# Celebrandil/CudaSift

Hardware: AMD Instinct MI355X
Metric: 1920x1080 SIFT frames/sec (higher is better)
Workload: dtype f32

## Files before the change

### cudasift_amd/csrc/chain.hpp

```cpp
#pragma once
#include "common.hpp"

#define CHAIN_MAX_LEVELS 3
struct ChainLevel { int w, h, p; long long off; };
struct ChainGeom {
  int K, T, tiles_x, tiles_y;
  long long frame_stride;
  ChainLevel lv[CHAIN_MAX_LEVELS + 1];
};

static inline int chain_lds_floats(int K, int T)
{
  const int n1 = ((T + 3) << (K - 1)) - 3, n0 = ((T + 3) << K) - 3;
  return n0 * n0 + n0 * n1 + n1 * n1;
}
#define CHAIN_LDS_FLOATS_MAX (85 * 85 + 85 * 41 + 41 * 41)
#define CHAIN_LDS_FLOATS_EMBED (53 * 53 + 53 * 25 + 25 * 25)

#ifdef __HIPCC__
__device__ __forceinline__ void scaledown_chain_block(float *__restrict__ scratch, const ChainGeom &G, const Taps5 &t,
                                                      int tile, int frame_index, float *lds)
{
  const int lane = threadIdx.x & 63, wave = threadIdx.x >> 6, nwaves = blockDim.x >> 6;
  const int tx = tile % G.tiles_x, ty = tile / G.tiles_x;
  float *frame = scratch + (long long)frame_index * G.frame_stride;
  const float k0 = t.k[0], k1 = t.k[1], k2 = t.k[2];
  auto ax = [&](int k) -> int { return (tx * G.T - 2) * (1 << (G.K - k)) + 2; };
  auto ay = [&](int k) -> int { return (ty * G.T - 2) * (1 << (G.K - k)) + 2; };
  auto n = [&](int k) -> int { return ((G.T + 3) << (G.K - k)) - 3; };
  float *const s_a = lds, *const s_h = lds + n(0) * n(0), *const s_b = s_h + n(0) * n(1);
  {
    const ChainLevel &S = G.lv[0];
    const float *src = frame + S.off;
    const int n0 = n(0), ax0 = ax(0), ay0 = ay(0);
// ... 56 lines not shown
```

### cudasift_amd/csrc/common.hpp

```cpp
#pragma once
#include <hip/hip_runtime.h>
#include <stdint.h>
#include <stddef.h>
#include "misift.h"

#define NUM_SCALES 5
#define NUM_BLURS  8
#define NUM_DOG    7
#define CNT_STRIDE 64
#define CNT_MAXPTS 17
#define CNT_CAND   20
#define CNT_CANDOVF 28
#define CNT_PTOVF  29
#define CNT_CHAINTMO 30
#define CNT_DET    32
#define CNT_DUP    40
#define CNT_SPARE_BLOCKS 9
#define CNT_BIG    48
#define CNT_TICKET 49
#define CNT_ORIDONE 50
#define CNT_FUSETMO 31

struct alignas(16) SiftPointD {
  float xpos, ypos, scale, sharpness, edgeness, orientation, score, ambiguity;
  int   match;
  float match_xpos, match_ypos, match_error, subsampling;
  float empty[3];
  float data[128];
};
static_assert(sizeof(SiftPointD) == MISIFT_POINT_BYTES, "record size");

struct BatchLayout {
  SiftPointD *recs;
  const int *counts, *offsets;
  int stride;
// ... 281 lines not shown
  float *d_own_scratch;
  size_t own_scratch_floats;
  int lds_pad_lpd, lds_pad_scan, lds_pad_orient, lds_pad_descr;
  float patch_reach;
  int fold_descr_tail;
  int descr_big_fallbacks;
  PendingBig pending_big;
  unsigned *d_refcap;
  size_t refcap_bytes;
  unsigned *d_capcnt;
  size_t capcnt_bytes;
  int refcap_limit;
  void *d_match_tmp;
  size_t match_tmp_bytes;
  int num_cus;
  int split_tail, in_capture;
  hipStream_t stream2;
  hipEvent_t ev_fork, ev_join;
  int *pack_counts, *pack_offsets;
  SiftPointD *pack_dst;
  int orient_blocks_per_cu;
  int point_blocks_per_cu;
  int strip_waves_per_cu, scan_waves_per_cu;
  int chain_max_frames;
  int chain_embed;
  unsigned chain_wait_ticks;
  int chain_fallbacks;
  int fuse_orient;
  unsigned fuse_wait_ticks;
  int fuse_fallbacks;
  int bin_min_frames;
  int small_frames;
  int lowpass_tile;
  int strip_rows_small;
  int scan_rows_small_coarse;
  int scan_rows_small;
  int cur_binned;
  int balance_frames;
  int cur_balanced;
  int4 *d_block_map;
// ... 131 lines not shown
```

### cudasift_amd/csrc/kernels_dog.hip

```cpp
#include <stdlib.h>
#include <string.h>
#include <math.h>
#include "common.hpp"
#include "chain.hpp"

#define WAVES_PER_BLOCK 4
#define OUT_LANES 62

struct ItemCoord { int frame, strip, seg; bool valid; };

__device__ __forceinline__ ItemCoord decode_item(const StripGeom &g)
{
  const unsigned lb = (g.noremap & 1) ? blockIdx.x : xcd_remap(blockIdx.x, gridDim.x);
  const int wave = __builtin_amdgcn_readfirstlane((int)(threadIdx.x >> 6));
  const long long item = (long long)lb * WAVES_PER_BLOCK + wave;
  const long long nitems = (long long)g.nframes * g.nstrips * g.nsegs;
  ItemCoord c;
  c.valid = item < nitems;
  if (g.noremap & 2) {
    c.strip = (int)(item % g.nstrips);
    const long long r = item / g.nstrips;
    c.seg = (int)(r % g.nsegs);
    c.frame = (int)(r / g.nsegs);
  } else {
// ... 840 lines not shown
  unsigned cap_clear_words;
  ScanOct o[MISIFT_MAX_OCTAVES];
};

#ifndef SCAN_OCC
#define SCAN_OCC (SCAN_RING ? 4 : 3)
#endif
#ifndef SCAN_STAMPS
#define SCAN_STAMPS 0
#endif
#if SCAN_STAMPS
#define STAMP_MAX(slot) do { if ((threadIdx.x & 63) == 0) atomicMax(&counters[(size_t)G.nframes * CNT_STRIDE + (slot)], (unsigned)wall_clock64()); } while (0)
#else
#define STAMP_MAX(slot) do { } while (0)
#endif
template <int FAST, bool CHAIN>
__global__ __launch_bounds__(256, SCAN_OCC) void dog_scan_all_kernel(const float *__restrict__ scratch, ScanAllGeom G,
                                                              AllTaps taps, float thresh,
                                                              unsigned *__restrict__ counters,
                                                              unsigned *__restrict__ cand, ChainGeom C, Taps5 k5,
                                                              int nchain)
{
  __shared__ v2f s_taps[WAVES_PER_BLOCK][NUM_SCAN_PAIRS * 5];
#if SCAN_RING
  __shared__ float4 s_win[WAVES_PER_BLOCK][RING_FLOAT4S];
  static_assert(sizeof(float4) * WAVES_PER_BLOCK * RING_FLOAT4S >= sizeof(float) * CHAIN_LDS_FLOATS_EMBED,
                "the chain borrows the scan's row ring");
#else
  __shared__ float s_chain_lds[CHAIN ? CHAIN_LDS_FLOATS_EMBED : 4];
#endif
// ... 6 lines not shown
  const int wave = __builtin_amdgcn_readfirstlane((int)(threadIdx.x >> 6));
  const int lane = threadIdx.x & 63;
  bool chain_failed = false;
  float4 *xch = nullptr;
#if SCAN_XCH && SCAN_XCH_DPP < 3
  if (lane < 4) s_xch[wave][(lane >> 1) * XCH_PLANE + (lane & 1) * (XCH_PLANE - 1)] = make_float4(0.f, 0.f, 0.f, 0.f);
  xch = &s_xch[wave][lane];
#endif
  if (CHAIN) {
#if SCAN_STAMPS
    if (blockIdx.x == 0 && threadIdx.x == 0) counters[(size_t)G.nframes * CNT_STRIDE + 8] = (unsigned)wall_clock64();
    if (threadIdx.x == 0) STAMP_MAX(14);
    if (threadIdx.x == 0 && lb + 1 == gridDim.x) STAMP_MAX(16);
    if (threadIdx.x == 0 && lb == (unsigned)nchain) STAMP_MAX(17);
#endif
    if (lb < (unsigned)nchain) {
      const int tiles = C.tiles_x * C.tiles_y;
#if SCAN_RING
      float *chain_lds = reinterpret_cast<float *>(&s_win[0][0]);
#else
      float *chain_lds = s_chain_lds;
#endif
      scaledown_chain_block(const_cast<float *>(scratch), C, k5, (int)(lb % tiles), (int)(lb / tiles), chain_lds);
      asm volatile("s_waitcnt vmcnt(0)" ::: "memory");
      __builtin_amdgcn_fence(__ATOMIC_RELEASE, "workgroup");
      __syncthreads();
      STAMP_MAX(9);
      if (threadIdx.x == 0) {
        unsigned *spare = counters + (size_t)G.nframes * CNT_STRIDE;
        const unsigned sub = lb & 15u, members = ((unsigned)nchain - sub + 15u) / 16u;
        if (atomicAdd(&spare[64 + 32 * sub], 1u) == members - 1u) {
          const unsigned nsub = (unsigned)nchain < 16u ? (unsigned)nchain : 16u;
          if (atomicAdd(&spare[32], 1u) == nsub - 1u && G.wait_ticks != 0u) {
            __hip_atomic_fetch_or(&spare[0], 0x80000000u, __ATOMIC_RELAXED, __HIP_MEMORY_SCOPE_AGENT);
            STAMP_MAX(18);
          }
        }
      }
      STAMP_MAX(19);
      return;
    }
    lb -= (unsigned)nchain;
    if (G.wait_lev < G.nlev && (long long)lb * WAVES_PER_BLOCK + (WAVES_PER_BLOCK - 1) >= G.o[G.wait_lev].item_begin) {
      STAMP_MAX(15);
      __shared__ unsigned s_chain_ok;
      if (threadIdx.x == 0) {
        const unsigned long long t0 = wall_clock64();
        unsigned ok = 1u;
        while ((__hip_atomic_fetch_add(&counters[(size_t)G.nframes * CNT_STRIDE], 1u, __ATOMIC_RELAXED, __HIP_MEMORY_SCOPE_AGENT) &
                0x80000000u) == 0u) {
          if (wall_clock64() - t0 > (unsigned long long)G.wait_ticks) { ok = 0u; break; }
          __builtin_amdgcn_s_sleep(8);
        }
        if (!ok) atomicAdd(&counters[CNT_CHAINTMO], 1u);
        s_chain_ok = ok;
      }
      __syncthreads();
      STAMP_MAX(13);
// ... 586 lines not shown
    const CapLayout L = cap_layout(P);
    const int rc = ensure_capcnt(ctx, P, L);
    if (rc) return rc;
    G.cap_clear = ctx->d_capcnt;
    G.cap_clear_words = L.words * (unsigned)P.nframes;
  }
  const AllTaps at = pack_taps(taps, P.noct);
  ChainGeom C;
  Taps5 t5;
  memset(&C, 0, sizeof(C));
  memset(&t5, 0, sizeof(t5));
  int nchain = 0;
  if (chain) {
    C = *chain;
    for (int j = 0; j < 5; j++) t5.k[j] = k5[j];
    nchain = C.tiles_x * C.tiles_y * P.nframes;
    G.wait_lev = 0;
    G.wait_ticks = ctx->chain_wait_ticks;
    for (int k = 0; k < G.nlev; k++)
      if (G.o[k].img_off == C.lv[0].off) G.wait_lev = k + 1;
  }
  const dim3 grid((unsigned)((items + WAVES_PER_BLOCK - 1) / WAVES_PER_BLOCK) + (unsigned)nchain);
  LaunchScope ls(ctx, "dog_scan");
#define SCAN_LAUNCH(F, CH) hipLaunchKernelGGL((dog_scan_all_kernel<F, CH>), grid, dim3(256), (size_t)ctx->lds_pad_scan, ctx->stream, scratch, G, at, \
                                              thresh, ctx->d_counters, ctx->d_cand, C, t5, nchain)
  if (chain) {
    if (fast && !ragged) SCAN_LAUNCH(1, true);
    else if (fast) SCAN_LAUNCH(2, true);
    else SCAN_LAUNCH(0, true);
  } else {
    if (fast && !ragged) SCAN_LAUNCH(1, false);
    else if (fast) SCAN_LAUNCH(2, false);
    else SCAN_LAUNCH(0, false);
  }
#undef SCAN_LAUNCH
// ... 41 lines not shown
```

### cudasift_amd/csrc/kernels_pyramid.hip

```cpp
#include <string.h>
#include "common.hpp"
#include "chain.hpp"

#define WAVES_PER_BLOCK 4
#define OUT_LANES 62

struct ItemCoord { int frame, strip, seg; bool valid; };

__device__ __forceinline__ ItemCoord decode_item(const StripGeom &g)
{
  const unsigned lb = (g.noremap & 1) ? blockIdx.x : xcd_remap(blockIdx.x, gridDim.x);
  const int wave = __builtin_amdgcn_readfirstlane((int)(threadIdx.x >> 6));
  const long long item = (long long)lb * WAVES_PER_BLOCK + wave;
  const long long nitems = (long long)g.nframes * g.nstrips * g.nsegs;
  ItemCoord c;
  c.valid = item < nitems;
  if (g.noremap & 2) {
    c.strip = (int)(item % g.nstrips);
    const long long r = item / g.nstrips;
    c.seg = (int)(r % g.nsegs);
    c.frame = (int)(r / g.nsegs);
  } else {
    c.seg = (int)(item % g.nsegs);
    const long long r = item / g.nsegs;
// ... 360 lines not shown
    const float *c = s_DH + (2 * Y) * (LPT_TW / 2) + X;
    float v = __builtin_fmaf(d2, c[2 * (LPT_TW / 2)], d0 * (c[0] + c[4 * (LPT_TW / 2)]));
    v = __builtin_fmaf(d1, c[LPT_TW / 2] + c[3 * (LPT_TW / 2)], v);
    LPT_STORE1(out2 + (size_t)Yg * dpitch2 + Xg, v);
  }
}

template <int FAST>
__global__ __launch_bounds__(256) void scaledown_kernel(const float *__restrict__ src, StripGeom g,
                                                        float *__restrict__ dst, int dpitch,
                                                        long long dst_frame_stride, Taps5 t, int src_aligned,
                                                        int dst_aligned)
{
  const ItemCoord it = decode_item(g);
  if (!it.valid) return;
  const int lane = threadIdx.x & 63;
  const int q = it.strip * OUT_LANES + lane - 1;
  const int w2 = g.width / 2, h2 = g.height / 2;
  const float *img = src + (long long)it.frame * g.frame_stride;
  float *out = dst + (long long)it.frame * dst_frame_stride;
  const int y0 = it.seg * g.seg_rows;
  const int y1 = min(y0 + g.seg_rows, h2);
  const float k0 = t.k[0], k1 = t.k[1], k2 = t.k[2];
  const bool sal = src_aligned != 0, dal = dst_aligned != 0;

  const QuadCol qa = make_quadcol(2 * q, g.width), qb = make_quadcol(2 * q + 1, g.width);
  struct Raw2 { float4 A, B; };
  auto ldraw = [&](int y) -> Raw2 {
    const float *row = img + (size_t)clampi(y, 0, g.height - 1) * g.pitch;
    Raw2 r;
    r.A = load_quad_t<FAST>(row, 2 * q, g.width, sal, qa);
    r.B = load_quad_t<FAST>(row, 2 * q + 1, g.width, sal, qb);
    return r;
  };
  auto hfilt = [&](const Raw2 &rw) -> float4 {
    const float4 A = rw.A, B = rw.B;
    const float lz = lane_from_left(B.z), lw = lane_from_left(B.w);
    const float rx = lane_from_right(A.x);
    float4 h;
    float s;
    s = __builtin_fmaf(k0, lz + A.z, k1 * (lw + A.y));  h.x = __builtin_fmaf(k2, A.x, s);
    s = __builtin_fmaf(k0, A.x + B.x, k1 * (A.y + A.w)); h.y = __builtin_fmaf(k2, A.z, s);
    s = __builtin_fmaf(k0, A.z + B.z, k1 * (A.w + B.y)); h.z = __builtin_fmaf(k2, B.x, s);
    s = __builtin_fmaf(k0, B.x + rx, k1 * (B.y + B.w)); h.w = __builtin_fmaf(k2, B.z, s);
    return h;
  };
  auto vcomb = [&](float a0, float a1, float a2, float a3, float a4) -> float {
    float s = __builtin_fmaf(k2, a2, k0 * (a0 + a4));
    s = __builtin_fmaf(k1, a1 + a3, s);
    return s;
  };

  auto hrow = [&](int y) -> float4 { return hfilt(ldraw(y)); };
  const bool writer = lane >= 1 && lane <= OUT_LANES && 4 * q < w2;
  const bool fast_store = FAST && (w2 & 3) == 0 && dal;
  float4 t0 = hrow(2 * y0 - 2), t1 = hrow(2 * y0 - 1), t2 = hrow(2 * y0), t3, t4;
  Raw2 ra = ldraw(2 * y0 + 1), rb = ldraw(2 * y0 + 2), rc = ldraw(2 * y0 + 3), rd = ldraw(2 * y0 + 4);
  for (int y = y0; y < y1; y++) {
    const Raw2 na = ldraw(2 * y + 5), nb = ldraw(2 * y + 6);
    t3 = hfilt(ra);
    t4 = hfilt(rb);
    ra = rc; rb = rd; rc = na; rd = nb;
    float4 o;
    o.x = vcomb(t0.x, t1.x, t2.x, t3.x, t4.x);
    o.y = vcomb(t0.y, t1.y, t2.y, t3.y, t4.y);
    o.z = vcomb(t0.z, t1.z, t2.z, t3.z, t4.z);
    o.w = vcomb(t0.w, t1.w, t2.w, t3.w, t4.w);
    if (writer) {
      if (fast_store) *reinterpret_cast<float4 *>(out + (size_t)y * dpitch + 4 * q) = o;
      else store_quad(out + (size_t)y * dpitch, q, w2, dal, o);
    }
    t0 = t2; t1 = t3; t2 = t4;
  }
}

__global__ __launch_bounds__(1024) void scaledown_chain_kernel(float *__restrict__ scratch, ChainGeom G, Taps5 t)
{
  __shared__ float s_lds[CHAIN_LDS_FLOATS_MAX];
  scaledown_chain_block(scratch, G, t, (int)blockIdx.x, (int)blockIdx.y, s_lds);
}

template <typename SRC>
__global__ __launch_bounds__(256) void scaleup_kernel(const SRC *__restrict__ src0, int w, int h, int spitch,
                                                      long long src_frame_stride, float *__restrict__ dst0, int dpitch,
                                                      long long dst_frame_stride)
{
  const int x = blockIdx.x * 64 + (threadIdx.x & 63);
  const int y = blockIdx.y * 4 + (threadIdx.x >> 6);
// ... 167 lines not shown
```

### cudasift_amd/csrc/misift_host.hip

```cpp
#include <stdarg.h>
#include <stdio.h>
#include <stdlib.h>
#include <string.h>
#include <math.h>
#include <initializer_list>
#include <map>
#include <mutex>
#include <string>
#include <utility>
#include <vector>
#include "common.hpp"
#include "chain.hpp"
#include "pair_plan.hpp"

static thread_local char g_err[512] = "";

void misift_set_error(const char *fmt, ...)
{
  va_list ap;
  va_start(ap, fmt);
  vsnprintf(g_err, sizeof(g_err), fmt, ap);
  va_end(ap);
}

// ... 260 lines not shown
  {"lds_pad_descr", "MISIFT_LDS_PAD_DESCR"}, {"lowpass_tile", "MISIFT_LOWPASS_TILE"}, {"strip_rows_small", "MISIFT_STRIP_ROWS_SMALL"},
  {"scan_rows_small_coarse", "MISIFT_SCAN_ROWS_SMALL_COARSE"}, {"scan_rows_small", "MISIFT_SCAN_ROWS_SMALL"},
  {"host_spin", "MISIFT_HOST_SPIN"}, {"refcap_limit", "MISIFT_TEST_REFCAP_LIMIT"}, {"fuse_orient", "MISIFT_FUSE_ORIENT"},
  {"fuse_wait_us", "MISIFT_FUSE_WAIT_US"},
};
static bool tunables_from_env()
{
  const char *e = getenv("MISIFT_TUNABLES");
  return e && atoi(e) != 0;
}
static int apply_knob(misift_ctx *ctx, const char *name, double v)
{
  const int i = (int)v;
  const auto is = [&](const char *n) { return strcmp(name, n) == 0; };
  if (is("graph")) extra(ctx)->graph_mode = i != 0;
  else if (is("split_tail")) ctx->split_tail = i;
  else if (is("bin")) ctx->bin_detections = i != 0;
  else if (is("descr_occ")) ctx->descr_occ = i;
  else if (is("tile")) ctx->tile_descr = ctx->tile_orient = i != 0;
  else if (is("tile_descr")) ctx->tile_descr = i != 0;
  else if (is("tile_orient")) ctx->tile_orient = i != 0;
  else if (is("orient_blocks")) ctx->orient_blocks_per_cu = i > 0 ? i : 6;
  else if (is("point_blocks")) ctx->point_blocks_per_cu = i > 0 ? i : 8;
  else if (is("strip_waves")) ctx->strip_waves_per_cu = i > 0 ? i : 16;
  else if (is("scan_waves")) ctx->scan_waves_per_cu = i > 0 ? i : 16;
  else if (is("chain_frames")) ctx->chain_max_frames = i;
  else if (is("chain_embed")) ctx->chain_embed = i != 0;
  else if (is("chain_wait_us")) ctx->chain_wait_ticks = (unsigned)(v * 100.0);
  else if (is("bin_min_frames")) ctx->bin_min_frames = i;
  else if (is("small_frames")) ctx->small_frames = i;
  else if (is("balance")) ctx->balance_frames = i != 0;
// ... 22 lines not shown
    for (const KnobName &k : KNOBS) all += std::string(all.empty() ? "" : ",") + k.name + "=" + k.env;
  return all.c_str();
}

extern "C" void misift_ctx_destroy(misift_ctx *ctx);
static int ctx_init(misift_ctx *ctx, CtxFull *f, int device, void *stream)
{
  ctx->device = device;
  ctx->stream = (hipStream_t)stream;
  default_options_full(&ctx->opt);
  hipDeviceProp_t prop;
  HIP_TRY(hipGetDeviceProperties(&prop, device));
  ctx->num_cus = prop.multiProcessorCount > 0 ? prop.multiProcessorCount : 256;
  ctx->strip_waves_per_cu = 32;
  ctx->scan_waves_per_cu = 32;
  ctx->split_tail = 8;
  {
    int lo = 0, hi = 0;
    HIP_TRY(hipDeviceGetStreamPriorityRange(&lo, &hi));
    HIP_TRY(hipStreamCreateWithPriority(&ctx->stream2, hipStreamNonBlocking, hi));
    HIP_TRY(hipEventCreateWithFlags(&ctx->ev_fork, hipEventDisableTiming));
    HIP_TRY(hipEventCreateWithFlags(&ctx->ev_join, hipEventDisableTiming));
  }
  ctx->bin_detections = 1;
  ctx->descr_occ = 4;
  ctx->tile_descr = 1;
  ctx->tile_orient = 0;
  ctx->orient_blocks_per_cu = 6;
  ctx->point_blocks_per_cu = 8;
  ctx->chain_max_frames = 4;
  ctx->chain_embed = 1;
  ctx->chain_wait_ticks = 10000000u;
  ctx->bin_min_frames = 4;
  ctx->small_frames = 4;
  ctx->balance_frames = 1;
  ctx->fold_descr_tail = 1;
  ctx->fuse_orient = 0;
  ctx->fuse_wait_ticks = 10000000u;
  ctx->patch_reach = 17.9f;
  ctx->refcap_limit = 32;
  ctx->lowpass_tile = 1;
  ctx->strip_rows_small = 6;
  ctx->scan_rows_small_coarse = 2;
  ctx->scan_rows_small = 4;
  ctx->host_spin = 0;
  if (tunables_from_env()) {
// ... 193 lines not shown
  if (x->d_mb_plan) misift_dev_free(x->d_mb_plan);
  if (ctx->d_counters) misift_dev_free(ctx->d_counters);
  if (ctx->h_counters) hipHostFree(ctx->h_counters);
  if (ctx->d_flags) misift_dev_free(ctx->d_flags);
  if (ctx->h_flags) hipHostFree(ctx->h_flags);
  if (ctx->d_cand) misift_dev_free(ctx->d_cand);
  if (ctx->d_det) misift_dev_free(ctx->d_det);
  if (ctx->d_det_sorted) misift_dev_free(ctx->d_det_sorted);
  if (ctx->d_block_map) misift_dev_free(ctx->d_block_map);
  if (ctx->d_own_scratch) misift_dev_free(ctx->d_own_scratch);
  if (ctx->d_match_tmp) misift_dev_free(ctx->d_match_tmp);
  if (ctx->d_refcap) misift_dev_free(ctx->d_refcap);
  if (ctx->d_capcnt) misift_dev_free(ctx->d_capcnt);
  if (ctx->ev0) hipEventDestroy(ctx->ev0);
  if (ctx->ev1) hipEventDestroy(ctx->ev1);
  if (ctx->stream2) { hipStreamSynchronize(ctx->stream2); hipStreamDestroy(ctx->stream2); }
  if (ctx->ev_fork) hipEventDestroy(ctx->ev_fork);
  if (ctx->ev_join) hipEventDestroy(ctx->ev_join);
  if (x->own_stream) hipStreamDestroy(x->own_stream);
  delete reinterpret_cast<CtxFull *>(ctx);
}

extern "C" int misift_ctx_set_graph_replay(misift_ctx *ctx, int on)
{
  ARG_CHECK(ctx != nullptr);
  extra(ctx)->graph_mode = on ? 1 : 0;
  return MISIFT_OK;
}

extern "C" int misift_ctx_set_stream(misift_ctx *ctx, void *stream)
{
  ARG_CHECK(ctx != nullptr);
  ctx->stream = (hipStream_t)stream;
// ... 555 lines not shown
      L.img_off = (long long)(lv[o].img - d_scratch);
      L.subsampling = (float)(1 << (num_octaves - o));
      L.lowest_scale = lowest_scale / L.subsampling;
      size_t c = (size_t)L.w * L.h / 4;
      if (c < 16384) c = 16384;
      L.cand_cap = (unsigned)c;
      L.cand_off = off;
      off += L.cand_cap;
      tapsv[o] = octave_taps(table, o);
    }
    rc = misift_ensure_frames(ctx, nframes, off);
    if (rc) return rc;
    rc = ensure_det(ctx, nframes, max_pts);
    if (rc) return rc;
  }
  bool scanned = false;
  if (ctx->opt.fused && ctx->split_tail && nframes >= ctx->split_tail && !ctx->in_capture && first_down_done &&
      num_octaves >= 3 && ctx->stream2) {
    HIP_TRY(hipEventRecord(ctx->ev_fork, ctx->stream));
    HIP_TRY(hipStreamWaitEvent(ctx->stream2, ctx->ev_fork, 0));
    rc = launch_dog_scan_all(ctx, d_scratch, P, tapsv.data(), thresh, 0, 2);
    if (rc) return rc;
    hipStream_t saved = ctx->stream;
    ctx->stream = ctx->stream2;
    for (int o = num_octaves - 1; o >= 2 && !rc; o--) {
      const Level &src = lv[o], &dst = lv[o - 1];
      StripGeom g = make_geom(ctx, src.w, src.h, src.p, nframes, SS, dst.w, dst.h, 62);
      rc = launch_scaledown(ctx, src.img, g, dst.img, dst.p, SS, k5);
    }
    if (!rc) rc = launch_dog_scan_all(ctx, d_scratch, P, tapsv.data(), thresh, 2, num_octaves);
    ctx->stream = saved;
    if (rc) return rc;
    HIP_TRY(hipEventRecord(ctx->ev_join, ctx->stream2));
    HIP_TRY(hipStreamWaitEvent(ctx->stream, ctx->ev_join, 0));
    scanned = true;
  }
  const bool chained = !scanned && !tiny && nframes <= ctx->chain_max_frames;
  ChainGeom embed;
  bool embedded = false;
  if (chained && ctx->opt.fused && ctx->chain_embed && ctx->want_export && first_down_done && num_octaves >= 3 &&
      num_octaves - 2 <= 3) {
    const int o = num_octaves - 1, nlev = o - 1;
    int dims[4][3];
    long long offs[4];
    for (int k = 0; k <= nlev; k++) {
      dims[k][0] = lv[o - k].w; dims[k][1] = lv[o - k].h; dims[k][2] = lv[o - k].p;
      offs[k] = (long long)(lv[o - k].img - d_scratch);
    }
    rc = make_chain_geom(&embed, SS, dims, offs, nlev, 4);
    if (rc) return rc;
    embedded = true;
  }
  for (int o = num_octaves; o >= 2 && !scanned && !embedded;) {
    if (o == num_octaves && first_down_done) { o--; continue; }
    if (chained) {
      const int nlev = (o - 1) < 3 ? (o - 1) : 3;
      int dims[4][3];
      long long offs[4];
      for (int k = 0; k <= nlev; k++) {
        dims[k][0] = lv[o - k].w; dims[k][1] = lv[o - k].h; dims[k][2] = lv[o - k].p;
        offs[k] = (long long)(lv[o - k].img - d_scratch);
      }
      rc = launch_scaledown_chain(ctx, d_scratch, SS, nframes, dims, offs, nlev, k5);
      if (rc) return rc;
      o -= nlev;
      continue;
    }
    const Level &src = lv[o], &dst = lv[o - 1];
    if (dst.w < 1 || dst.h < 1) break;
    StripGeom g = make_geom(ctx, src.w, src.h, src.p, nframes, SS, dst.w, dst.h, 62);
    rc = launch_scaledown(ctx, src.img, g, dst.img, dst.p, SS, k5);
    if (rc) return rc;
    o--;
  }
  if (ctx->opt.fused) {
    if (!scanned) {
      rc = launch_dog_scan_all(ctx, d_scratch, P, tapsv.data(), thresh, 0, num_octaves, embedded ? &embed : nullptr, k5);
      if (rc) return rc;
    }
    rc = launch_refine_all(ctx, d_scratch, P, tapsv.data(), thresh, 10.0f, 1.0f / NUM_SCALES, max_pts);
    if (rc) return rc;
    const bool binned = (ctx->bin_detections && nframes >= ctx->bin_min_frames) || ctx->opt.deterministic;
    ctx->cur_binned = binned ? 1 : 0;
    ctx->cur_balanced = 0;
    if (binned) {
      rc = launch_bin_detections(ctx, P, max_pts);
      if (rc) return rc;
    }
    if (ctx->fuse_orient && !binned && !ctx->pack_dst && nframes <= ctx->small_frames && ctx->tile_descr && !ctx->tile_orient &&
        !ctx->in_capture)
      return launch_orient_descr_fused(ctx, d_scratch, P, pts, max_pts);
    rc = launch_orient_all(ctx, d_scratch, P, pts, max_pts);
    if (rc) return rc;
    if (ctx->opt.deterministic) {
// ... 78 lines not shown
    if (ctx->pending_big.valid) {
      bool any = false;
      for (int f = 0; f < nframes; f++) any = any || ctx->h_counters[(size_t)f * CNT_STRIDE + CNT_BIG] != 0;
      if (!any) ctx->pending_big.valid = 0;
      else {
        rc = launch_descr_big_pending(ctx);
        if (!rc) rc = wait_host_flag(ctx, ctx->h_counters + (size_t)nframes * CNT_STRIDE, ctx->export_seq);
        if (rc) return rc;
      }
    }
  } else {
    HIP_TRY(hipMemcpyAsync(ctx->h_counters, ctx->d_counters, sizeof(unsigned) * CNT_STRIDE * (size_t)nframes,
                           hipMemcpyDeviceToHost, ctx->stream));
    HIP_TRY(hipStreamSynchronize(ctx->stream));
  }
  if (ctx->h_counters[CNT_CHAINTMO]) return MISIFT_RETRY_CHAIN;
  if (ctx->h_counters[CNT_FUSETMO]) return MISIFT_RETRY_FUSE;
  const int slot = 2 * num_octaves + (ctx->opt.fix_numpts ? 1 : 0);
  for (int f = 0; f < nframes; f++) {
    const unsigned c = ctx->h_counters[(size_t)f * CNT_STRIDE + slot];
    num_pts_out[f] = (int)(c < (unsigned)max_pts ? c : (unsigned)max_pts);
    if (ctx->h_counters[(size_t)f * CNT_STRIDE + CNT_CANDOVF]) *cand_overflow = true;
  }
  return MISIFT_OK;
}

static int enqueue_via_graph(misift_ctx *ctx, const CallKey &key, const void *d_imgs, long long frame_stride,
                             float *d_scratch, SiftPointD *pts)
{
  CtxExtra *x = extra(ctx);
  if (!x->graph_mode || ctx->profile || !d_scratch || key.scale_up || !key.fused) return 0;
// ... 851 lines not shown
```

### cudasift_amd/csrc/pipeline.hip

```cpp
#include <string.h>
#include <vector>
#include "common.hpp"

__global__ __launch_bounds__(1024) void export_counts_kernel(const unsigned *__restrict__ counters, int nframes, int slot,
                                                              int max_pts, int *__restrict__ counts,
                                                              int *__restrict__ offsets, int staged_noct)
{
  __shared__ int wave_tot[16];
  __shared__ int carry_s;
  const int tid = threadIdx.x, lane = tid & 63, wave = tid >> 6;
  if (tid == 0) carry_s = 0;
  __syncthreads();
  for (int f0 = 0; f0 < nframes; f0 += 1024) {
    const int f = f0 + tid;
    int c = 0;
    if (f < nframes) {
      const unsigned *cnt = counters + (size_t)f * CNT_STRIDE;
      unsigned n = cnt[slot];
      if (staged_noct > 0) {
        n = 0;
        for (int k = 1; k <= staged_noct; k++) {
          n += cnt[CNT_DET + k];
          if (k < staged_noct || (slot & 1)) n += cnt[CNT_DUP + k];
        }
      }
      c = (int)(n < (unsigned)max_pts ? n : (unsigned)max_pts);
      counts[f] = cnt[CNT_CANDOVF] ? -1 : c;
      if (cnt[CNT_CANDOVF]) c = 0;
    }
    if (!offsets) continue;
    int incl = c;
    for (int d = 1; d < 64; d <<= 1) {
      const int o = __shfl_up(incl, d, 64);
      if (lane >= d) incl += o;
    }
    if (lane == 63) wave_tot[wave] = incl;
    __syncthreads();
    int base = carry_s;
    for (int w = 0; w < wave; w++) base += wave_tot[w];
    if (f < nframes) offsets[f] = base + incl - c;
    __syncthreads();
    if (tid == 1023) carry_s = base + incl;
    __syncthreads();
// ... 159 lines not shown
    misift_set_error("misift_pipe_submit: invalid argument");
    return MISIFT_EINVAL;
  }
  if (p->submitted - p->collected >= p->depth) {
    misift_set_error("misift_pipe_submit: all %d slots are in flight — collect a batch first", p->depth);
    return MISIFT_EINVAL;
  }
  misift_ctx *ctx = p->ctx;
  HIP_TRY(hipSetDevice(ctx->device));
  PipeSlot &s = p->slots[p->submitted % p->depth];
  const size_t elem = p->src_u8 ? 1 : sizeof(float);
  HIP_TRY(hipMemcpyAsync(s.d_frames, host_frames, elem * p->frame_elems * nframes, hipMemcpyHostToDevice, p->s_up));
  HIP_TRY(hipEventRecord(s.ev_uploaded, p->s_up));
  HIP_TRY(hipStreamWaitEvent(p->s_compute, s.ev_uploaded, 0));
  hipStream_t saved = ctx->stream;
  const int saved_split = ctx->split_tail;
  ctx->stream = p->s_compute;
  ctx->split_tail = 0;
  const int fused_saved = ctx->opt.fused;
  if (misift_tiny_call(p->width, p->height, p->num_octaves)) ctx->opt.fused = 0;
  int rc = misift_extract_enqueue(ctx, s.d_frames, p->src_u8, nframes, (long long)p->frame_elems, p->width, p->height,
                                  p->width, p->num_octaves, p->init_blur, p->thresh, p->lowest_scale, 0, p->d_scratch,
                                  p->d_pts, p->max_pts);
  if (!rc) rc = launch_export_counts(ctx, nframes, p->num_octaves, p->max_pts, s.d_counts, s.d_counts + p->batch);
  if (!rc) rc = launch_pack_records(ctx, p->d_pts, p->max_pts, nframes, s.d_counts + p->batch, s.d_packed);
  ctx->stream = saved;
  ctx->split_tail = saved_split;
  ctx->opt.fused = fused_saved;
  if (rc) return rc;
  HIP_TRY(hipEventRecord(s.ev_done, p->s_compute));
  HIP_TRY(hipStreamWaitEvent(p->s_down, s.ev_done, 0));
  HIP_TRY(hipMemcpyAsync(s.h_counts, s.d_counts, sizeof(int) * (2 * (size_t)p->batch + 1), hipMemcpyDeviceToHost,
                         p->s_down));
  HIP_TRY(hipEventRecord(s.ev_counts, p->s_down));
  s.nframes = nframes;
  p->submitted++;
  return MISIFT_OK;
}

extern "C" int misift_pipe_collect(misift_pipe *p, int *nframes_out, int *counts_out, void *host_records,
                                   size_t capacity_records, size_t *nrecords_out)
{
// ... 72 lines not shown
```

Before: 58000.

## Embed staged scaledown chain into DoG scan launch, replacing second-stream split tail

Removes the two-stream split-tail path that forked the lower-octave scaledowns and scans onto a high-priority stream. For large batches it now embeds the lower-octave scaledowns as extra workgroups in the first DoG scan launch. These workgroups run in stages, and each stage waits on per-frame completion flags and tickets before reading the level above it. The scaledown body is factored into a shared device function with a write-through store variant. This removes separate kernel launches and event syncs, at the cost of spin-waiting workgroups, a timeout fallback reported per frame, and a dependence on workgroup scheduling order.

```diff
diff --git a/cudasift_amd/csrc/chain.hpp b/cudasift_amd/csrc/chain.hpp
--- a/cudasift_amd/csrc/chain.hpp
+++ b/cudasift_amd/csrc/chain.hpp
@@ -3,11 +3,17 @@
 
 #define CHAIN_MAX_LEVELS 3
 struct ChainLevel { int w, h, p; long long off; };
+struct ChainStage { int nstrips, nsegs, seg_rows; unsigned wg_begin; };
 struct ChainGeom {
   int K, T, tiles_x, tiles_y;
+  int staged;
+  int nwg;
   long long frame_stride;
   ChainLevel lv[CHAIN_MAX_LEVELS + 1];
+  ChainStage st[CHAIN_MAX_LEVELS];
 };
+#define CHAIN_FLAG_DONE 0x80000000u
+#define CHAIN_FLAG_FAILED 0x40000000u
 
 static inline int chain_lds_floats(int K, int T)
 {
@@ -18,6 +24,87 @@
 #define CHAIN_LDS_FLOATS_EMBED (53 * 53 + 53 * 25 + 25 * 25)
 
 #ifdef __HIPCC__
+#define SD_OUT_LANES 62
+typedef float sd_v4f __attribute__((ext_vector_type(4)));
+template <bool WT>
+__device__ __forceinline__ void sd_store1(float *p, float v)
+{
+  if (WT) __hip_atomic_store(p, v, __ATOMIC_RELAXED, __HIP_MEMORY_SCOPE_AGENT);
+  else *p = v;
+}
+template <int FAST, bool WT>
+__device__ __forceinline__ void scaledown_item(const float *__restrict__ img, int width, int height, int pitch,
+                                               float *__restrict__ out, int dpitch, int strip, int y0, int y1,
+                                               const Taps5 &t, bool sal, bool dal)
+{
+  const int lane = threadIdx.x & 63;
+  const int q = strip * SD_OUT_LANES + lane - 1;
+  const int w2 = width / 2;
+  const float k0 = t.k[0], k1 = t.k[1], k2 = t.k[2];
+
+  const QuadCol qa = make_quadcol(2 * q, width), qb = make_quadcol(2 * q + 1, width);
+  struct Raw2 { float4 A, B; };
+  auto ldraw = [&](int y) -> Raw2 {
+    const float *row = img + (size_t)clampi(y, 0, height - 1) * pitch;
+    Raw2 r;
+    r.A = load_quad_t<FAST>(row, 2 * q, width, sal, qa);
+    r.B = load_quad_t<FAST>(row, 2 * q + 1, width, sal, qb);
+    return r;
+  };
+  auto hfilt = [&](const Raw2 &rw) -> float4 {
+    const float4 A = rw.A, B = rw.B;
+    const float lz = lane_from_left(B.z), lw = lane_from_left(B.w);
+    const float rx = lane_from_right(A.x);
+    float4 h;
+    float s;
+    s = __builtin_fmaf(k0, lz + A.z, k1 * (lw + A.y));  h.x = __builtin_fmaf(k2, A.x, s);
+    s = __builtin_fmaf(k0, A.x + B.x, k1 * (A.y + A.w)); h.y = __builtin_fmaf(k2, A.z, s);
+    s = __builtin_fmaf(k0, A.z + B.z, k1 * (A.w + B.y)); h.z = __builtin_fmaf(k2, B.x, s);
+    s = __builtin_fmaf(k0, B.x + rx, k1 * (B.y + B.w)); h.w = __builtin_fmaf(k2, B.z, s);
+    return h;
+  };
+  auto vcomb = [&](float a0, float a1, float a2, float a3, float a4) -> float {
+    float s = __builtin_fmaf(k2, a2, k0 * (a0 + a4));
+    s = __builtin_fmaf(k1, a1 + a3, s);
+    return s;
+  };
+
+  auto hrow = [&](int y) -> float4 { return hfilt(ldraw(y)); };
+  const bool writer = lane >= 1 && lane <= SD_OUT_LANES && 4 * q < w2;
+  const bool fast_store = FAST && (w2 & 3) == 0 && dal;
+  float4 t0 = hrow(2 * y0 - 2), t1 = hrow(2 * y0 - 1), t2 = hrow(2 * y0), t3, t4;
+  Raw2 ra = ldraw(2 * y0 + 1), rb = ldraw(2 * y0 + 2), rc = ldraw(2 * y0 + 3), rd = ldraw(2 * y0 + 4);
+  for (int y = y0; y < y1; y++) {
+    const Raw2 na = ldraw(2 * y + 5), nb = ldraw(2 * y + 6);
+    t3 = hfilt(ra);
+    t4 = hfilt(rb);
+    ra = rc; rb = rd; rc = na; rd = nb;
+    float4 o;
+    o.x = vcomb(t0.x, t1.x, t2.x, t3.x, t4.x);
+    o.y = vcomb(t0.y, t1.y, t2.y, t3.y, t4.y);
+    o.z = vcomb(t0.z, t1.z, t2.z, t3.z, t4.z);
+    o.w = vcomb(t0.w, t1.w, t2.w, t3.w, t4.w);
+    if (writer) {
+      float *row = out + (size_t)y * dpitch;
+      const int x = 4 * q;
+      if (fast_store || (dal && x + 3 < w2)) {
+        if (WT) {
+          const sd_v4f w = {o.x, o.y, o.z, o.w};
+          asm volatile("global_store_dwordx4 %0, %1, off sc1\n\ts_nop 1" ::"v"(reinterpret_cast<sd_v4f *>(row + x)), "v"(w) : "memory");
+        } else {
+          *reinterpret_cast<float4 *>(row + x) = o;
+        }
+      } else {
+        if (x < w2) sd_store1<WT>(row + x, o.x);
+        if (x + 1 < w2) sd_store1<WT>(row + x + 1, o.y);
+        if (x + 2 < w2) sd_store1<WT>(row + x + 2, o.z);
+        if (x + 3 < w2) sd_store1<WT>(row + x + 3, o.w);
+      }
+    }
+    t0 = t2; t1 = t3; t2 = t4;
+  }
+}
+
 __device__ __forceinline__ void scaledown_chain_block(float *__restrict__ scratch, const ChainGeom &G, const Taps5 &t,
                                                       int tile, int frame_index, float *lds)
 {
diff --git a/cudasift_amd/csrc/common.hpp b/cudasift_amd/csrc/common.hpp
--- a/cudasift_amd/csrc/common.hpp
+++ b/cudasift_amd/csrc/common.hpp
@@ -19,6 +19,8 @@
 #define CNT_BIG    48
 #define CNT_TICKET 49
 #define CNT_ORIDONE 50
+#define CNT_CHAIN_TICKET 58
+#define CNT_CHAIN_FLAG 61
 #define CNT_FUSETMO 31
 
 struct alignas(16) SiftPointD {
@@ -330,9 +332,7 @@
   void *d_match_tmp;
   size_t match_tmp_bytes;
   int num_cus;
-  int split_tail, in_capture;
-  hipStream_t stream2;
-  hipEvent_t ev_fork, ev_join;
+  int in_capture;
   int *pack_counts, *pack_offsets;
   SiftPointD *pack_dst;
   int orient_blocks_per_cu;
@@ -340,6 +340,7 @@
   int strip_waves_per_cu, scan_waves_per_cu;
   int chain_max_frames;
   int chain_embed;
+  int embed_batches;
   unsigned chain_wait_ticks;
   int chain_fallbacks;
   int fuse_orient;
diff --git a/cudasift_amd/csrc/kernels_dog.hip b/cudasift_amd/csrc/kernels_dog.hip
--- a/cudasift_amd/csrc/kernels_dog.hip
+++ b/cudasift_amd/csrc/kernels_dog.hip
@@ -878,6 +878,58 @@
 #else
 #define STAMP_MAX(slot) do { } while (0)
 #endif
+__device__ __forceinline__ bool chain_wait_flag(unsigned *flag, unsigned wait_ticks)
+{
+  unsigned ok = 1u;
+  if ((threadIdx.x & 63) == 0) {
+    const unsigned long long t0 = wall_clock64();
+    for (;;) {
+      const unsigned v = __hip_atomic_fetch_add(flag, 1u, __ATOMIC_RELAXED, __HIP_MEMORY_SCOPE_AGENT);
+      if (v & CHAIN_FLAG_DONE) { ok = (v & CHAIN_FLAG_FAILED) ? 0u : 1u; break; }
+      if (wall_clock64() - t0 > (unsigned long long)wait_ticks) { ok = 0u; break; }
+      __builtin_amdgcn_s_sleep(8);
+    }
+  }
+  ok = (unsigned)__builtin_amdgcn_readfirstlane((int)ok);
+  __builtin_amdgcn_fence(__ATOMIC_ACQUIRE, "workgroup");
+  return ok != 0u;
+}
+
+__device__ __forceinline__ void chain_stage_item(float *__restrict__ scratch, const ChainGeom &C, const Taps5 &k5, unsigned lb,
+                                                 int wave, int nframes, unsigned wait_ticks, unsigned *__restrict__ counters)
+{
+  int s = 0;
+  for (int k = 1; k < C.K; k++)
+    if (lb >= C.st[k].wg_begin) s = k;
+  s = __builtin_amdgcn_readfirstlane(s);
+  const int nstrips = C.st[s].nstrips, nsegs = C.st[s].nsegs, seg_rows = C.st[s].seg_rows;
+  const long long item = (long long)(lb - C.st[s].wg_begin) * WAVES_PER_BLOCK + wave;
+  const int per_frame = nstrips * nsegs;
+  if (item >= (long long)per_frame * nframes) return;
+  const int strip = (int)(item % nstrips);
+  const long long r = item / nstrips;
+  const int seg = (int)(r % nsegs), frame = (int)(r / nsegs);
+  unsigned *cnt = counters + (size_t)frame * CNT_STRIDE;
+  bool ok = true;
+  if (s > 0) ok = chain_wait_flag(cnt + CNT_CHAIN_FLAG + s - 1, wait_ticks);
+  if (ok) {
+    const ChainLevel &S = C.lv[s], &D = C.lv[s + 1];
+    float *fr = scratch + (long long)frame * C.frame_stride;
+    const int y0 = seg * seg_rows, y1 = min(y0 + seg_rows, D.h);
+    if ((S.w & 3) == 0) scaledown_item<1, true>(fr + S.off, S.w, S.h, S.p, fr + D.off, D.p, strip, y0, y1, k5, true, true);
+    else scaledown_item<2, true>(fr + S.off, S.w, S.h, S.p, fr + D.off, D.p, strip, y0, y1, k5, true, true);
+    asm volatile("s_waitcnt vmcnt(0)" ::: "memory");
+  }
+  if ((threadIdx.x & 63) == 0) {
+    if (!ok) {
+      atomicAdd(&cnt[CNT_CHAINTMO], 1u);
+      __hip_atomic_fetch_or(&cnt[CNT_CHAIN_FLAG + s], CHAIN_FLAG_DONE | CHAIN_FLAG_FAILED, __ATOMIC_RELAXED, __HIP_MEMORY_SCOPE_AGENT);
+    } else if (atomicAdd(&cnt[CNT_CHAIN_TICKET + s], 1u) == (unsigned)per_frame - 1u && wait_ticks != 0u) {
+      __hip_atomic_fetch_or(&cnt[CNT_CHAIN_FLAG + s], CHAIN_FLAG_DONE, __ATOMIC_RELAXED, __HIP_MEMORY_SCOPE_AGENT);
+    }
+  }
+}
+
 template <int FAST, bool CHAIN>
 __global__ __launch_bounds__(256, SCAN_OCC) void dog_scan_all_kernel(const float *__restrict__ scratch, ScanAllGeom G,
                                                               AllTaps taps, float thresh,
@@ -914,7 +966,11 @@
     if (threadIdx.x == 0 && lb + 1 == gridDim.x) STAMP_MAX(16);
     if (threadIdx.x == 0 && lb == (unsigned)nchain) STAMP_MAX(17);
 #endif
-    if (lb < (unsigned)nchain) {
+    if (C.staged && lb < (unsigned)nchain) {
+      chain_stage_item(const_cast<float *>(scratch), C, k5, lb, wave, G.nframes, G.wait_ticks, counters);
+      return;
+    }
+    if (!C.staged && lb < (unsigned)nchain) {
       const int tiles = C.tiles_x * C.tiles_y;
 #if SCAN_RING
       float *chain_lds = reinterpret_cast<float *>(&s_win[0][0]);
@@ -941,7 +997,8 @@
       return;
     }
     lb -= (unsigned)nchain;
-    if (G.wait_lev < G.nlev && (long long)lb * WAVES_PER_BLOCK + (WAVES_PER_BLOCK - 1) >= G.o[G.wait_lev].item_begin) {
+    if (!C.staged && G.wait_lev < G.nlev &&
+        (long long)lb * WAVES_PER_BLOCK + (WAVES_PER_BLOCK - 1) >= G.o[G.wait_lev].item_begin) {
       STAMP_MAX(15);
       __shared__ unsigned s_chain_ok;
       if (threadIdx.x == 0) {
@@ -1558,11 +1615,15 @@
   if (chain) {
     C = *chain;
     for (int j = 0; j < 5; j++) t5.k[j] = k5[j];
-    nchain = C.tiles_x * C.tiles_y * P.nframes;
+    nchain = C.staged ? C.nwg : C.tiles_x * C.tiles_y * P.nframes;
     G.wait_lev = 0;
     G.wait_ticks = ctx->chain_wait_ticks;
     for (int k = 0; k < G.nlev; k++)
       if (G.o[k].img_off == C.lv[0].off) G.wait_lev = k + 1;
+    if (C.staged && G.wait_lev < G.nlev) {
+      misift_set_error("dog_scan_all: a level the staged chain writes cannot be scanned by the launch that carries it");
+      return MISIFT_EINVAL;
+    }
   }
   const dim3 grid((unsigned)((items + WAVES_PER_BLOCK - 1) / WAVES_PER_BLOCK) + (unsigned)nchain);
   LaunchScope ls(ctx, "dog_scan");
diff --git a/cudasift_amd/csrc/kernels_pyramid.hip b/cudasift_amd/csrc/kernels_pyramid.hip
--- a/cudasift_amd/csrc/kernels_pyramid.hip
+++ b/cudasift_amd/csrc/kernels_pyramid.hip
@@ -398,64 +398,12 @@
 {
   const ItemCoord it = decode_item(g);
   if (!it.valid) return;
-  const int lane = threadIdx.x & 63;
-  const int q = it.strip * OUT_LANES + lane - 1;
-  const int w2 = g.width / 2, h2 = g.height / 2;
-  const float *img = src + (long long)it.frame * g.frame_stride;
-  float *out = dst + (long long)it.frame * dst_frame_stride;
+  const int h2 = g.height / 2;
   const int y0 = it.seg * g.seg_rows;
-  const int y1 = min(y0 + g.seg_rows, h2);
-  const float k0 = t.k[0], k1 = t.k[1], k2 = t.k[2];
-  const bool sal = src_aligned != 0, dal = dst_aligned != 0;
-
-  const QuadCol qa = make_quadcol(2 * q, g.width), qb = make_quadcol(2 * q + 1, g.width);
-  struct Raw2 { float4 A, B; };
-  auto ldraw = [&](int y) -> Raw2 {
-    const float *row = img + (size_t)clampi(y, 0, g.height - 1) * g.pitch;
-    Raw2 r;
-    r.A = load_quad_t<FAST>(row, 2 * q, g.width, sal, qa);
-    r.B = load_quad_t<FAST>(row, 2 * q + 1, g.width, sal, qb);
-    return r;
-  };
-  auto hfilt = [&](const Raw2 &rw) -> float4 {
-    const float4 A = rw.A, B = rw.B;
-    const float lz = lane_from_left(B.z), lw = lane_from_left(B.w);
-    const float rx = lane_from_right(A.x);
-    float4 h;
-    float s;
-    s = __builtin_fmaf(k0, lz + A.z, k1 * (lw + A.y));  h.x = __builtin_fmaf(k2, A.x, s);
-    s = __builtin_fmaf(k0, A.x + B.x, k1 * (A.y + A.w)); h.y = __builtin_fmaf(k2, A.z, s);
-    s = __builtin_fmaf(k0, A.z + B.z, k1 * (A.w + B.y)); h.z = __builtin_fmaf(k2, B.x, s);
-    s = __builtin_fmaf(k0, B.x + rx, k1 * (B.y + B.w)); h.w = __builtin_fmaf(k2, B.z, s);
-    return h;
-  };
-  auto vcomb = [&](float a0, float a1, float a2, float a3, float a4) -> float {
-    float s = __builtin_fmaf(k2, a2, k0 * (a0 + a4));
-    s = __builtin_fmaf(k1, a1 + a3, s);
-    return s;
-  };
-
-  auto hrow = [&](int y) -> float4 { return hfilt(ldraw(y)); };
-  const bool writer = lane >= 1 && lane <= OUT_LANES && 4 * q < w2;
-  const bool fast_store = FAST && (w2 & 3) == 0 && dal;
-  float4 t0 = hrow(2 * y0 - 2), t1 = hrow(2 * y0 - 1), t2 = hrow(2 * y0), t3, t4;
-  Raw2 ra = ldraw(2 * y0 + 1), rb = ldraw(2 * y0 + 2), rc = ldraw(2 * y0 + 3), rd = ldraw(2 * y0 + 4);
-  for (int y = y0; y < y1; y++) {
-    const Raw2 na = ldraw(2 * y + 5), nb = ldraw(2 * y + 6);
-    t3 = hfilt(ra);
-    t4 = hfilt(rb);
-    ra = rc; rb = rd; rc = na; rd = nb;
-    float4 o;
-    o.x = vcomb(t0.x, t1.x, t2.x, t3.x, t4.x);
-    o.y = vcomb(t0.y, t1.y, t2.y, t3.y, t4.y);
-    o.z = vcomb(t0.z, t1.z, t2.z, t3.z, t4.z);
-    o.w = vcomb(t0.w, t1.w, t2.w, t3.w, t4.w);
-    if (writer) {
-      if (fast_store) *reinterpret_cast<float4 *>(out + (size_t)y * dpitch + 4 * q) = o;
-      else store_quad(out + (size_t)y * dpitch, q, w2, dal, o);
-    }
-    t0 = t2; t1 = t3; t2 = t4;
-  }
+  static_assert(SD_OUT_LANES == OUT_LANES, "launch_scaledown's geometry is built for OUT_LANES quads per strip");
+  scaledown_item<FAST, false>(src + (long long)it.frame * g.frame_stride, g.width, g.height, g.pitch,
+                              dst + (long long)it.frame * dst_frame_stride, dpitch, it.strip, y0, min(y0 + g.seg_rows, h2), t,
+                              src_aligned != 0, dst_aligned != 0);
 }
 
 __global__ __launch_bounds__(1024) void scaledown_chain_kernel(float *__restrict__ scratch, ChainGeom G, Taps5 t)
diff --git a/cudasift_amd/csrc/misift_host.hip b/cudasift_amd/csrc/misift_host.hip
--- a/cudasift_amd/csrc/misift_host.hip
+++ b/cudasift_amd/csrc/misift_host.hip
@@ -298,7 +298,7 @@
   const int i = (int)v;
   const auto is = [&](const char *n) { return strcmp(name, n) == 0; };
   if (is("graph")) extra(ctx)->graph_mode = i != 0;
-  else if (is("split_tail")) ctx->split_tail = i;
+  else if (is("split_tail")) ctx->embed_batches = i != 0;
   else if (is("bin")) ctx->bin_detections = i != 0;
   else if (is("descr_occ")) ctx->descr_occ = i;
   else if (is("tile")) ctx->tile_descr = ctx->tile_orient = i != 0;
@@ -351,14 +351,6 @@
   ctx->num_cus = prop.multiProcessorCount > 0 ? prop.multiProcessorCount : 256;
   ctx->strip_waves_per_cu = 32;
   ctx->scan_waves_per_cu = 32;
-  ctx->split_tail = 8;
-  {
-    int lo = 0, hi = 0;
-    HIP_TRY(hipDeviceGetStreamPriorityRange(&lo, &hi));
-    HIP_TRY(hipStreamCreateWithPriority(&ctx->stream2, hipStreamNonBlocking, hi));
-    HIP_TRY(hipEventCreateWithFlags(&ctx->ev_fork, hipEventDisableTiming));
-    HIP_TRY(hipEventCreateWithFlags(&ctx->ev_join, hipEventDisableTiming));
-  }
   ctx->bin_detections = 1;
   ctx->descr_occ = 4;
   ctx->tile_descr = 1;
@@ -367,6 +359,7 @@
   ctx->point_blocks_per_cu = 8;
   ctx->chain_max_frames = 4;
   ctx->chain_embed = 1;
+  ctx->embed_batches = 1;
   ctx->chain_wait_ticks = 10000000u;
   ctx->bin_min_frames = 4;
   ctx->small_frames = 4;
@@ -590,9 +583,6 @@
   if (ctx->d_capcnt) misift_dev_free(ctx->d_capcnt);
   if (ctx->ev0) hipEventDestroy(ctx->ev0);
   if (ctx->ev1) hipEventDestroy(ctx->ev1);
-  if (ctx->stream2) { hipStreamSynchronize(ctx->stream2); hipStreamDestroy(ctx->stream2); }
-  if (ctx->ev_fork) hipEventDestroy(ctx->ev_fork);
-  if (ctx->ev_join) hipEventDestroy(ctx->ev_join);
   if (x->own_stream) hipStreamDestroy(x->own_stream);
   delete reinterpret_cast<CtxFull *>(ctx);
 }
@@ -1178,32 +1168,33 @@
     rc = ensure_det(ctx, nframes, max_pts);
     if (rc) return rc;
   }
-  bool scanned = false;
-  if (ctx->opt.fused && ctx->split_tail && nframes >= ctx->split_tail && !ctx->in_capture && first_down_done &&
-      num_octaves >= 3 && ctx->stream2) {
-    HIP_TRY(hipEventRecord(ctx->ev_fork, ctx->stream));
-    HIP_TRY(hipStreamWaitEvent(ctx->stream2, ctx->ev_fork, 0));
-    rc = launch_dog_scan_all(ctx, d_scratch, P, tapsv.data(), thresh, 0, 2);
-    if (rc) return rc;
-    hipStream_t saved = ctx->stream;
-    ctx->stream = ctx->stream2;
-    for (int o = num_octaves - 1; o >= 2 && !rc; o--) {
-      const Level &src = lv[o], &dst = lv[o - 1];
-      StripGeom g = make_geom(ctx, src.w, src.h, src.p, nframes, SS, dst.w, dst.h, 62);
-      rc = launch_scaledown(ctx, src.img, g, dst.img, dst.p, SS, k5);
-    }
-    if (!rc) rc = launch_dog_scan_all(ctx, d_scratch, P, tapsv.data(), thresh, 2, num_octaves);
-    ctx->stream = saved;
-    if (rc) return rc;
-    HIP_TRY(hipEventRecord(ctx->ev_join, ctx->stream2));
-    HIP_TRY(hipStreamWaitEvent(ctx->stream, ctx->ev_join, 0));
-    scanned = true;
-  }
-  const bool chained = !scanned && !tiny && nframes <= ctx->chain_max_frames;
+  const bool chained = !tiny && nframes <= ctx->chain_max_frames;
   ChainGeom embed;
   bool embedded = false;
+  if (!chained && !tiny && ctx->opt.fused && ctx->chain_embed && ctx->embed_batches && !ctx->in_capture && first_down_done &&
+      num_octaves >= 3 && num_octaves - 2 <= CHAIN_MAX_LEVELS && (((uintptr_t)d_scratch) & 15) == 0 && (SS & 3) == 0) {
+    const int o = num_octaves - 1, nlev = o - 1;
+    memset(&embed, 0, sizeof(embed));
+    embed.K = nlev; embed.staged = 1; embed.frame_stride = SS;
+    bool ok = true;
+    unsigned wg = 0;
+    for (int k = 0; k <= nlev; k++) {
+      const Level &L = lv[o - k];
+      embed.lv[k].w = L.w; embed.lv[k].h = L.h; embed.lv[k].p = L.p; embed.lv[k].off = (long long)(L.img - d_scratch);
+      if (L.w < 1 || L.h < 1 || (L.p & 3) != 0 || (embed.lv[k].off & 3) != 0) ok = false;
+    }
+    for (int k = 0; k < nlev && ok; k++) {
+      const Level &src = lv[o - k], &dst = lv[o - k - 1];
+      const StripGeom g = make_geom(ctx, src.w, src.h, src.p, nframes, SS, dst.w, dst.h, 62);
+      embed.st[k].nstrips = g.nstrips; embed.st[k].nsegs = g.nsegs; embed.st[k].seg_rows = g.seg_rows;
+      embed.st[k].wg_begin = wg;
+      wg += (unsigned)(((long long)nframes * g.nstrips * g.nsegs + 3) / 4);
+    }
+    embed.nwg = (int)wg;
+    embedded = ok;
+  }
   if (chained && ctx->opt.fused && ctx->chain_embed && ctx->want_export && first_down_done && num_octaves >= 3 &&
-      num_octaves - 2 <= 3) {
+      num_octaves - 2 <= CHAIN_MAX_LEVELS) {
     const int o = num_octaves - 1, nlev = o - 1;
     int dims[4][3];
     long long offs[4];
@@ -1215,7 +1206,7 @@
     if (rc) return rc;
     embedded = true;
   }
-  for (int o = num_octaves; o >= 2 && !scanned && !embedded;) {
+  for (int o = num_octaves; o >= 2 && !embedded;) {
     if (o == num_octaves && first_down_done) { o--; continue; }
     if (chained) {
       const int nlev = (o - 1) < 3 ? (o - 1) : 3;
@@ -1238,10 +1229,13 @@
     o--;
   }
   if (ctx->opt.fused) {
-    if (!scanned) {
+    if (embedded && embed.staged) {
+      rc = launch_dog_scan_all(ctx, d_scratch, P, tapsv.data(), thresh, 0, 2, &embed, k5);
+      if (!rc) rc = launch_dog_scan_all(ctx, d_scratch, P, tapsv.data(), thresh, 2, num_octaves);
+    } else {
       rc = launch_dog_scan_all(ctx, d_scratch, P, tapsv.data(), thresh, 0, num_octaves, embedded ? &embed : nullptr, k5);
-      if (rc) return rc;
-    }
+    }
+    if (rc) return rc;
     rc = launch_refine_all(ctx, d_scratch, P, tapsv.data(), thresh, 10.0f, 1.0f / NUM_SCALES, max_pts);
     if (rc) return rc;
     const bool binned = (ctx->bin_detections && nframes >= ctx->bin_min_frames) || ctx->opt.deterministic;
@@ -1350,7 +1344,8 @@
                            hipMemcpyDeviceToHost, ctx->stream));
     HIP_TRY(hipStreamSynchronize(ctx->stream));
   }
-  if (ctx->h_counters[CNT_CHAINTMO]) return MISIFT_RETRY_CHAIN;
+  for (int f = 0; f < nframes; f++)
+    if (ctx->h_counters[(size_t)f * CNT_STRIDE + CNT_CHAINTMO]) return MISIFT_RETRY_CHAIN;
   if (ctx->h_counters[CNT_FUSETMO]) return MISIFT_RETRY_FUSE;
   const int slot = 2 * num_octaves + (ctx->opt.fix_numpts ? 1 : 0);
   for (int f = 0; f < nframes; f++) {
diff --git a/cudasift_amd/csrc/pipeline.hip b/cudasift_amd/csrc/pipeline.hip
--- a/cudasift_amd/csrc/pipeline.hip
+++ b/cudasift_amd/csrc/pipeline.hip
@@ -25,8 +25,9 @@
         }
       }
       c = (int)(n < (unsigned)max_pts ? n : (unsigned)max_pts);
-      counts[f] = cnt[CNT_CANDOVF] ? -1 : c;
-      if (cnt[CNT_CANDOVF]) c = 0;
+      const bool bad = cnt[CNT_CANDOVF] != 0u || cnt[CNT_CHAINTMO] != 0u;
+      counts[f] = bad ? -1 : c;
+      if (bad) c = 0;
     }
     if (!offsets) continue;
     int incl = c;
@@ -216,9 +217,7 @@
   HIP_TRY(hipEventRecord(s.ev_uploaded, p->s_up));
   HIP_TRY(hipStreamWaitEvent(p->s_compute, s.ev_uploaded, 0));
   hipStream_t saved = ctx->stream;
-  const int saved_split = ctx->split_tail;
   ctx->stream = p->s_compute;
-  ctx->split_tail = 0;
   const int fused_saved = ctx->opt.fused;
   if (misift_tiny_call(p->width, p->height, p->num_octaves)) ctx->opt.fused = 0;
   int rc = misift_extract_enqueue(ctx, s.d_frames, p->src_u8, nframes, (long long)p->frame_elems, p->width, p->height,
@@ -227,7 +226,6 @@
   if (!rc) rc = launch_export_counts(ctx, nframes, p->num_octaves, p->max_pts, s.d_counts, s.d_counts + p->batch);
   if (!rc) rc = launch_pack_records(ctx, p->d_pts, p->max_pts, nframes, s.d_counts + p->batch, s.d_packed);
   ctx->stream = saved;
-  ctx->split_tail = saved_split;
   ctx->opt.fused = fused_saved;
   if (rc) return rc;
   HIP_TRY(hipEventRecord(s.ev_done, p->s_compute));
```

Measured after the change: 58590 (median of 4 runs). About the same (+1.0%).
